# engcang/FAST-LIO-SAM-QN

Measured on AMD Instinct MI355X. Metric: scan-pair registrations/sec on 100k-pt clouds, higher is better.
Workload: dtype f32 search / f64 accumulate

## Files before the change

fast-lio-sam-qn_amd/csrc/qn_knn_hist.cuh:

```cuda
#pragma once
#include "qn_device.cuh"
#include <type_traits>

namespace qn {

#define QN_HB 64
#define QN_HW (QN_HB + 5)
template <int HCAP>
struct WaveLdsH {
  WaveLds s;
  union alignas(16) {
    uint32_t hist[16][QN_HW];
    unsigned long long list[16][HCAP + 1];
    uint4 zero_[(16 * QN_HW + 3) / 4];
  } u;
  uint32_t cnt[16];
  uint32_t kth[16];
  alignas(16) uint32_t tile_sc[64 * 4];
};

typedef float qn_f4v __attribute__((ext_vector_type(4)));
#define QN_MM_FAR 1.0e15f
#define QN_MM_NCH 4
static_assert(QN_MM_NCH == 4, "tile_sc holds 64 x QN_MM_NCH words and is cleared with one 16-byte store per lane; the hit masks are two 32-bit words");
__device__ __forceinline__ uint32_t stage_chunk_mm(const GridView& g, WaveLds* lds, uint32_t* __restrict__ sc_out, const uint32_t cb, const uint32_t total,
                                                   const float Ox, const float Oy, const float Oz, float& c2max, const int j) {
  const int lane = threadIdx.x & 63;
  const uint32_t slot = cb + lane;
  float4 rel = make_float4(QN_MM_FAR, 0.f, 0.f, QN_MM_FAR * QN_MM_FAR); uint32_t sc = 63u << 26;
  if (slot < total) {
    const uint32_t sidx = lds->seg_start[j] + (slot - lds->seg_excl[j]);
    sc = sidx | (lds->seg_cid[j] << 26);
    const float4 p = g.pts[sidx];
    rel.x = p.x - Ox; rel.y = p.y - Oy; rel.z = p.z - Oz; rel.w = (rel.x * rel.x + rel.y * rel.y) + rel.z * rel.z;
    c2max = fmaxf(c2max, rel.w);
  }
  wave_lds_fence();
  lds->tile[lane] = rel; sc_out[lane] = sc;
  wave_lds_fence();
  return min(64u, total - cb);
}

template <int HCAP, bool MM = true>
__device__ __forceinline__ int wave_knn_hist(const GridView& g, float qx, float qy, float qz, bool active, float& r, int k, int max_rounds,
                                             WaveLdsH<HCAP>* L, int32_t* __restrict__ idx_base, float* __restrict__ d2_base, const uint32_t row) {
  const int lane = threadIdx.x & 63, qs = lane & 15, sub = lane >> 4;
  WaveLds* lds = &L->s;
  const int cx = cell_coord(qx, g.ox, g.inv_cell, g.nx);
  const int cy = cell_coord(qy, g.oy, g.inv_cell, g.ny);
  const int cz = cell_coord(qz, g.oz, g.inv_cell, g.nz);
  const float INF = __int_as_float(0x7f800000);
  int status = active ? 1 : 0;
  unsigned long long todo = __ballot(active);
  for (int round = 0; todo != 0 && round < max_rounds; round++) {
    const bool mine = (todo >> lane) & 1ull;
    uint32_t cid; int ncl; uint32_t nseg_all;
    build_clusters<4>(g, lds, todo, cx, cy, cz, qx, qy, qz, r, cid, ncl, nseg_all);
    { uint4* hz = (uint4*)&L->u.hist[0][0];
#pragma unroll
      for (int e = 0; e < (16 * QN_HW + 3) / 4; e += 64) if (e + lane < (16 * QN_HW + 3) / 4) hz[e + lane] = make_uint4(0u, 0u, 0u, 0u); }
    wave_lds_fence();
    const int base = (int)(__float_as_uint(4.f * r * r) >> 20) - (QN_HB - 2);
    const bool one_cluster = ncl == 1;
    const int base1 = mine ? base : -(1 << 28);
    uint32_t ncand;
    float Ox = 0.f, Oy = 0.f, Oz = 0.f, bsel = 0.f, q2 = 0.f, c2max = 0.f;
    if constexpr (MM) {
      const int l0 = __ffsll((long long)todo) - 1;
      Ox = rdlane(qx, l0); Oy = rdlane(qy, l0); Oz = rdlane(qz, l0);
      const float rx = qx - Ox, ry = qy - Oy, rz = qz - Oz;
      q2 = (rx * rx + ry * ry) + rz * rz;
      bsel = sub == 0 ? -2.f * rx : (sub == 1 ? -2.f * ry : (sub == 2 ? -2.f * rz : 1.f));
    }
    const float* tilef = (const float*)&lds->tile[0];
    const qn_f4v cin = {q2, q2, q2, q2};
    auto mm_groups = [&](const float (&av)[4], const uint32_t cnt, auto&& per_group) __attribute__((always_inline)) {
      qn_f4v d = __builtin_amdgcn_mfma_f32_16x16x4f32(av[0], bsel, cin, 0, 0, 0);
#pragma unroll
      for (int gi = 0; gi < 4; gi++) {
        qn_f4v dn = d;
        if (gi < 3) dn = __builtin_amdgcn_mfma_f32_16x16x4f32(av[gi + 1], bsel, cin, 0, 0, 0);
        if ((uint32_t)(16 * gi) < cnt) per_group(gi, d);
        d = dn;
      }
    };
    auto load_av = [&](float (&av)[4]) __attribute__((always_inline)) {
#pragma unroll
      for (int gi = 0; gi < 4; gi++) av[gi] = tilef[(16 * gi + qs) * 4 + sub];
    };
    const bool cached = nseg_all <= 64u && one_cluster;
    float avc[QN_MM_NCH][4];
    if constexpr (MM) {
      auto p1_group = [&](const uint32_t* __restrict__ scb, const int gi, const qn_f4v d) __attribute__((always_inline)) {
        if (one_cluster) {
#pragma unroll
          for (int e = 0; e < 4; e++) {
            const int bin = min(max((__float_as_int(d[e]) >> 20) - base1, 0), QN_HB - 1);
            atomicAdd(&L->u.hist[qs][bin], 1u);
          }
        } else {
          const uint4 cc = *(const uint4*)&scb[16 * gi + 4 * sub];
          const uint32_t ccv[4] = {cc.x >> 26, cc.y >> 26, cc.z >> 26, cc.w >> 26};
#pragma unroll
          for (int e = 0; e < 4; e++) {
            const int bin = max((__float_as_int(d[e]) >> 20) - base, 0);
            const bool ok = mine && ccv[e] == cid && bin < QN_HB - 1;
            atomicAdd(&L->u.hist[qs][ok ? bin : QN_HB + sub], 1u);
          }
        }
      };
      ncand = stream_tables<false>(g, lds, ncl, nseg_all, [&](const uint32_t total) __attribute__((always_inline)) {
        uint32_t cb0 = 0u;
        if (cached) {
          ((uint4*)L->tile_sc)[lane] = make_uint4(0u, 0u, 0u, 0u);
          wave_lds_fence();
          { const uint32_t ex = lds->seg_excl[lane], nx = lane < 63 ? lds->seg_excl[(lane + 1) & 63] : total;
            if (nx > ex && ex < 64u * QN_MM_NCH) L->tile_sc[ex] = (uint32_t)lane + 1u; }
          wave_lds_fence();
          uint32_t carry = 0u;
#pragma unroll
          for (int c = 0; c < QN_MM_NCH; c++) {
            if ((uint32_t)(64 * c) < total) {
              const uint32_t mk = max(wave_incl_max_u32(L->tile_sc[64 * c + lane]), carry);
              carry = rdlane(mk, 63);
              const uint32_t cnt = stage_chunk_mm(g, lds, L->tile_sc + 64 * c, 64u * c, total, Ox, Oy, Oz, c2max, (int)mk - 1);
              load_av(avc[c]);
              mm_groups(avc[c], cnt, [&](const int, const qn_f4v d) __attribute__((always_inline)) {
#pragma unroll
                for (int e = 0; e < 4; e++) atomicAdd(&L->u.hist[qs][min(max((__float_as_int(d[e]) >> 20) - base1, 0), QN_HB - 1)], 1u);
              });
            }
          }
          cb0 = 64u * QN_MM_NCH;
        }
        const uint32_t exs = lds->seg_excl[lane], nxs = lane < 63 ? lds->seg_excl[(lane + 1) & 63] : total;
        for (uint32_t cb = cb0; cb < total; cb += 64) {
          const int jg = chunk_segment(lds->tile_cid, cb, exs, nxs);
          const uint32_t cnt = stage_chunk_mm(g, lds, lds->tile_cid, cb, total, Ox, Oy, Oz, c2max, jg);
          float av[4]; load_av(av);
          mm_groups(av, cnt, [&](const int gi, const qn_f4v d) __attribute__((always_inline)) { p1_group(lds->tile_cid, gi, d); });
        }
      });
    } else {
    auto bin_of = [&](const float4& cp) __attribute__((always_inline)) { return max((int)(__float_as_uint(sqdist(qx, qy, qz, cp.x, cp.y, cp.z)) >> 20) - base, 0); };
    ncand = one_cluster
      ? stream_clusters<4>(g, lds, ncl, nseg_all, [&](const float4& cp, bool, uint32_t) __attribute__((always_inline)) {
          const int bin = min(max((int)(__float_as_uint(sqdist(qx, qy, qz, cp.x, cp.y, cp.z)) >> 20) - base1, 0), QN_HB - 1);
          atomicAdd(&L->u.hist[qs][bin], 1u);
        })
      : stream_clusters<4>(g, lds, ncl, nseg_all, [&](const float4& cp, bool in_tile, uint32_t ccid) __attribute__((always_inline)) {
          const int bin = bin_of(cp);
          const bool ok = mine && in_tile && ccid == cid && bin < QN_HB - 1;
          atomicAdd(&L->u.hist[qs][ok ? bin : QN_HB + sub], 1u);
        });
    }
    wave_lds_fence();
    uint32_t hv[16], mysum = 0;
#pragma unroll
    for (int j = 0; j < 16; j++) { hv[j] = L->u.hist[qs][sub * 16 + j]; if (j == 15 && sub == 3) hv[j] = 0u; mysum += hv[j]; }
    const uint32_t s0 = __shfl(mysum, qs), s1 = __shfl(mysum, qs + 16), s2 = __shfl(mysum, qs + 32), s3 = __shfl(mysum, qs + 48);
    uint32_t run = (sub > 0 ? s0 : 0u) + (sub > 1 ? s1 : 0u) + (sub > 2 ? s2 : 0u);
    const bool enough = s0 + s1 + s2 + s3 >= (uint32_t)k;
    int cross = 1 << 20;
#pragma unroll
    for (int j = 0; j < 16; j++) { run += hv[j]; if (cross == (1 << 20) && run >= (uint32_t)k) cross = sub * 16 + j; }
    cross = min(cross, __shfl_xor(cross, 16)); cross = min(cross, __shfl_xor(cross, 32));
    const uint32_t tau_bits = (uint32_t)(base + cross + 1) << 20;
    wave_lds_fence();
    if (lane < 16) { L->cnt[lane] = 0; L->kth[lane] = 0x7f800000u; }
    { uint4* lz = (uint4*)&L->u.list[0][0];
      constexpr int NZ = (int)(sizeof(L->u.list) / 16);
      static_assert(sizeof(L->u.list) % 16 == 0, "list rows are cleared with 16-byte stores");
#pragma unroll
      for (int e = 0; e < NZ; e += 64) if (e + lane < NZ) lz[e + lane] = make_uint4(0xffffffffu, 0xffffffffu, 0xffffffffu, 0xffffffffu); }
    wave_lds_fence();
    const bool collect = mine && enough;
    if constexpr (MM) {
      const float R2 = wave_max_f(fmaxf(c2max, mine ? q2 : 0.f));
      const float thr = collect ? (__uint_as_float(tau_bits) + 2.f * (R2 * 1.52587890625e-5f)) * 1.000001f : -__int_as_float(0x7f800000);
      float dummy = 0.f;
      const uint32_t cidm = cid;
      if (cached) {
        uint32_t mw[QN_MM_NCH / 2] = {0u, 0u};
#pragma unroll
        for (int c = 0; c < QN_MM_NCH; c++) {
          uint32_t& m = mw[c >> 1];
          if ((uint32_t)(64 * c) < ncand) {
            const uint32_t cnt = min(64u, ncand - 64u * c);
            qn_f4v d = __builtin_amdgcn_mfma_f32_16x16x4f32(avc[c][0], bsel, cin, 0, 0, 0);
#pragma unroll
            for (int gi = 0; gi < 4; gi++) {
              qn_f4v dn = d;
              if (gi < 3) dn = __builtin_amdgcn_mfma_f32_16x16x4f32(avc[c][gi + 1], bsel, cin, 0, 0, 0);
#pragma unroll
              for (int e = 0; e < 4; e++) m = __builtin_amdgcn_alignbit(m, __float_as_uint(d[e] - thr), 31);
              d = dn;
            }
          } else m <<= 16;
        }
        const uint32_t cntl = (uint32_t)(__popc(mw[0]) + __popc(mw[1]));
        const uint32_t h0 = __shfl(cntl, qs), h1 = __shfl(cntl, qs + 16), h2 = __shfl(cntl, qs + 32), h3 = __shfl(cntl, qs + 48);
        uint32_t pos = (sub > 0 ? h0 : 0u) + (sub > 1 ? h1 : 0u) + (sub > 2 ? h2 : 0u);
        if (sub == 0) L->cnt[qs] = h0 + h1 + h2 + h3;
        while (__any((mw[0] | mw[1]) != 0u)) {
          const bool lo = mw[0] != 0u;
          uint32_t w = lo ? mw[0] : mw[1];
          if (w != 0u) {
            const uint32_t I = (uint32_t)__clz((int)w);
            const uint32_t at = (lo ? 0u : 128u) + ((I >> 4) << 6) + (((I >> 2) & 3u) << 4) + 4u * (uint32_t)sub + (I & 3u);
            if (pos < HCAP) L->u.list[qs][pos] = (unsigned long long)(L->tile_sc[at] & 0x03ffffffu);
            pos++;
            w &= ~(0x80000000u >> I);
            if (lo) mw[0] = w; else mw[1] = w;
          }
        }
        wave_lds_fence();
      }
      if (!cached || ncand > 64u * QN_MM_NCH) {
      stream_tables<true>(g, lds, ncl, nseg_all, [&](const uint32_t total) __attribute__((always_inline)) {
        const uint32_t exs = lds->seg_excl[lane], nxs = lane < 63 ? lds->seg_excl[(lane + 1) & 63] : total;
        for (uint32_t cb = cached ? 64u * QN_MM_NCH : 0u; cb < total; cb += 64) {
          const int jg = chunk_segment(lds->tile_cid, cb, exs, nxs);
          const uint32_t cnt = stage_chunk_mm(g, lds, lds->tile_cid, cb, total, Ox, Oy, Oz, dummy, jg);
          float av[4]; load_av(av);
          mm_groups(av, cnt, [&](const int gi, const qn_f4v d) __attribute__((always_inline)) {
            bool hit[4];
#pragma unroll
            for (int e = 0; e < 4; e++) hit[e] = d[e] < thr;
            const uint4 cc = *(const uint4*)&lds->tile_cid[16 * gi + 4 * sub];
            if (!one_cluster) { hit[0] = hit[0] && (cc.x >> 26) == cidm; hit[1] = hit[1] && (cc.y >> 26) == cidm; hit[2] = hit[2] && (cc.z >> 26) == cidm; hit[3] = hit[3] && (cc.w >> 26) == cidm; }
            const uint32_t scv[4] = {cc.x, cc.y, cc.z, cc.w};
            if (hit[0] || hit[1] || hit[2] || hit[3]) {
#pragma unroll
              for (int e = 0; e < 4; e++) if (hit[e]) {
                const uint32_t pos = atomicAdd(&L->cnt[qs], 1u);
                if (pos < HCAP) L->u.list[qs][pos] = (unsigned long long)(scv[e] & 0x03ffffffu);
              }
            }
          });
        }
      }, ncand);
      }
      wave_lds_fence();
      const uint32_t Pn = min(L->cnt[qs], (uint32_t)HCAP);
      const int pmax = wave_max_i(collect ? (int)Pn : 0);
#pragma unroll
      for (int j = 0; j < HCAP / 4; j++) {
        if (4 * j >= pmax) break;
        const uint32_t slot = (uint32_t)(sub + 4 * j);
        if (collect && slot < Pn) {
          const float4 p = g.pts[(uint32_t)L->u.list[qs][slot]];
          L->u.list[qs][slot] = pack_key(sqdist(qx, qy, qz, p.x, p.y, p.z), __float_as_uint(p.w));
        }
      }
    } else {
    auto collect_one = [&](const float4& cp) __attribute__((always_inline)) {
      const float d2 = sqdist(qx, qy, qz, cp.x, cp.y, cp.z);
      if (collect && __float_as_uint(d2) < tau_bits) {
        const uint32_t pos = atomicAdd(&L->cnt[qs], 1u);
        if (pos < HCAP) L->u.list[qs][pos] = pack_key(d2, __float_as_uint(cp.w));
      }
    };
    if (one_cluster) stream_clusters<4, true>(g, lds, ncl, nseg_all, [&](const float4& cp, bool, uint32_t) __attribute__((always_inline)) { collect_one(cp); }, ncand);
    else stream_clusters<4, true>(g, lds, ncl, nseg_all, [&](const float4& cp, bool in_tile, uint32_t ccid) __attribute__((always_inline)) { if (in_tile && ccid == cid) collect_one(cp); }, ncand);
    }
    wave_lds_fence();
    const uint32_t P = L->cnt[qs];
    const bool ok = collect && P <= HCAP;
    const int maxP = wave_max_i(ok ? (int)P : 0);
    unsigned long long own[HCAP / 4]; int rank[HCAP / 4];
#pragma unroll
    for (int j = 0; j < HCAP / 4; j++) { own[j] = L->u.list[qs][sub + 4 * j]; rank[j] = 0; }
    auto rank_pass = [&](auto NJ) __attribute__((always_inline)) {
      for (int f = 0; f < maxP; f += 4) {
        unsigned long long kf[4];
#pragma unroll
        for (int u = 0; u < 4; u++) kf[u] = L->u.list[qs][min(f + u, HCAP)];
#pragma unroll
        for (int u = 0; u < 4; u++) {
#pragma unroll
          for (int j = 0; j < decltype(NJ)::value; j++) rank[j] += kf[u] < own[j] ? 1 : 0;
        }
      }
    };
    if (HCAP > 32 && maxP > 32) rank_pass(std::integral_constant<int, HCAP / 4>());
    else if (maxP > 28) rank_pass(std::integral_constant<int, 8>());
    else if (maxP > 24) rank_pass(std::integral_constant<int, 7>());
    else rank_pass(std::integral_constant<int, 6>());
#pragma unroll
    for (int j = 0; j < HCAP / 4; j++) if (own[j] != QN_INF_KEY && rank[j] == k - 1) L->kth[qs] = (uint32_t)(own[j] >> 32);
    wave_lds_fence();
    const float kth_d2 = __uint_as_float(L->kth[qs]);
    if (g.dbg && lane == 0) { atomicAdd(&g.dbg[0], (uint32_t)ncl); atomicAdd(&g.dbg[1], ncand); }
    bool retry = false;
    if (mine) {
      const int* b = lds->box[cid];
      const int ex0 = b[0], ex1 = b[1], ey0 = b[2], ey1 = b[3], ez0 = b[4], ez1 = b[5];
      float d = INF;
      if (ex0 > 0) d = fminf(d, qx - (g.ox + ex0 * g.cell));
      if (ex1 < g.nx - 1) d = fminf(d, (g.ox + (ex1 + 1) * g.cell) - qx);
      if (ey0 > 0) d = fminf(d, qy - (g.oy + ey0 * g.cell));
      if (ey1 < g.ny - 1) d = fminf(d, (g.oy + (ey1 + 1) * g.cell) - qy);
      if (ez0 > 0) d = fminf(d, qz - (g.oz + ez0 * g.cell));
      if (ez1 < g.nz - 1) d = fminf(d, (g.oz + (ez1 + 1) * g.cell) - qz);
      const bool whole = d == INF || !(r == r);
      if (!enough) {
        if (whole) status = 2;
        else {
          const uint32_t tot = s0 + s1 + s2 + s3;
          if (4u * tot < (uint32_t)k) {
            int kk = k; asm volatile("" : "+s"(kk));
            r = tot > 0 ? 2.f * r * sqrtf((float)kk / (float)tot) * 1.1f : 4.f * r + g.cell;
          } else { r = 2.f * r + g.cell; retry = true; }
        }
      } else if (!ok) status = 2;
      else {
        d -= g.eps;
        if (whole || (d > 0.f && kth_d2 < d * d)) {
          status = 0;
          uint32_t row_l = row; asm volatile("" : "+v"(row_l));
          int32_t* __restrict__ idx_out = idx_base + (size_t)row_l * k; float* __restrict__ d2_out = d2_base ? d2_base + (size_t)row_l * k : nullptr;
#pragma unroll
          for (int j = 0; j < HCAP / 4; j++) if (own[j] != QN_INF_KEY && rank[j] < k) {
            idx_out[rank[j]] = (int32_t)key_idx(own[j]);
            if (d2_out) d2_out[rank[j]] = key_d2(own[j]);
          }
        } else { r = fmaxf(sqrtf(kth_d2) * 1.000001f + g.eps, r + g.eps); retry = true; }
      }
    }
    todo = __ballot(retry && round + 1 < max_rounds);
    if (g.dbg && lane == 0 && todo) atomicAdd(&g.dbg[3], (uint32_t)__popcll(todo));
  }
  return status;
}


#define QN_HCAP1 128
struct WaveLdsH1 {
  WaveLds s;
  uint32_t hist[QN_HB];
  unsigned long long list[QN_HCAP1];
  uint32_t cnt, kth;
  unsigned long long best;
  uint32_t second, pad;
};

__device__ __forceinline__ int wave_knn_single(const GridView& g, float qx, float qy, float qz, float r, int k, WaveLdsH1* L,
                                               int32_t* __restrict__ idx_out, float* __restrict__ d2_out) {
  const int lane = threadIdx.x & 63;
  const float INF = __int_as_float(0x7f800000);
  if (!(qx == qx) || !(qy == qy) || !(qz == qz) || !(r == r)) return 2;
  const CapBox cap = cap_of(g, qx, qy, qz);
  if (cap.S > 0.f) r = fmaxf(r, sqrtf(cap.S) + 0.5f * g.cell);
  const float r_in = r;
  for (int round = 0; round < 64; round++) {
    const float rx = cap_extent(g, cap, r, 0), ry = cap_extent(g, cap, r, 1), rz = cap_extent(g, cap, r, 2);
    int x0 = rfl(cell_coord(qx - rx, g.ox, g.inv_cell, g.nx)), x1 = rfl(cell_coord(qx + rx, g.ox, g.inv_cell, g.nx));
    int y0 = rfl(cell_coord(qy - ry, g.oy, g.inv_cell, g.ny)), y1 = rfl(cell_coord(qy + ry, g.oy, g.inv_cell, g.ny));
    int z0 = rfl(cell_coord(qz - rz, g.oz, g.inv_cell, g.nz)), z1 = rfl(cell_coord(qz + rz, g.oz, g.inv_cell, g.nz));
    const bool tile_mode = ((x1 >> 3) - (x0 >> 3) + 1) * (y1 - y0 + 1) * (z1 - z0 + 1) > 128;
    if (tile_mode) {
      x0 = (x0 >> 3) << 3; x1 = min(((x1 >> 3) << 3) + 7, g.nx - 1);
      y0 = (y0 >> 2) << 2; y1 = min(((y1 >> 2) << 2) + 3, g.ny - 1);
      z0 = (z0 >> 2) << 2; z1 = min(((z1 >> 2) << 2) + 3, g.nz - 1);
    }
    wave_lds_fence();
    L->hist[lane] = 0; if (lane == 0) { L->cnt = 0; L->kth = 0x7f800000u; }
    wave_lds_fence();
    const int base = (int)(__float_as_uint(4.f * r * r) >> 20) - (QN_HB - 2);
    stream_box(g, x0, x1, y0, y1, z0, z1, tile_mode, &L->s, [&](const float4& p, bool valid, uint32_t) __attribute__((always_inline)) {
      const int bin = max((int)(__float_as_uint(sqdist(qx, qy, qz, p.x, p.y, p.z)) >> 20) - base, 0);
      if (valid && bin < QN_HB - 1) atomicAdd(&L->hist[bin], 1u);
    });
    wave_lds_fence();
    const uint32_t hv = lane < QN_HB - 1 ? L->hist[lane] : 0u;
    const uint32_t cum = wave_incl_scan_u32(hv, lane);
    const uint32_t total = rdlane(cum, 63);
    const bool enough = total >= (uint32_t)k;
    const unsigned long long reach = __ballot(cum >= (uint32_t)k);
    const int cross = reach ? __ffsll((long long)reach) - 1 : QN_HB - 2;
    uint32_t tau_bits = (uint32_t)(base + cross + 1) << 20;
    if (enough && rdlane(cum, cross) > (uint32_t)QN_HCAP1 && cross > 0) {
      const uint32_t below = rdlane(cum, cross - 1), need = (uint32_t)k - below;
      const uint32_t hi20 = (uint32_t)(base + cross);
      wave_lds_fence();
      L->hist[lane] = 0;
      wave_lds_fence();
      stream_box(g, x0, x1, y0, y1, z0, z1, tile_mode, &L->s, [&](const float4& p, bool valid, uint32_t) __attribute__((always_inline)) {
        const uint32_t bits = __float_as_uint(sqdist(qx, qy, qz, p.x, p.y, p.z));
        if (valid && (bits >> 20) == hi20) atomicAdd(&L->hist[(bits >> 14) & 63u], 1u);
      });
      wave_lds_fence();
      const uint32_t cum2 = wave_incl_scan_u32(L->hist[lane], lane);
      const unsigned long long reach2 = __ballot(cum2 >= need);
      const int sub = reach2 ? __ffsll((long long)reach2) - 1 : 63;
      tau_bits = (hi20 << 20) + ((uint32_t)(sub + 1) << 14);
    }
    float d = INF;
    if (x0 > 0) d = fminf(d, cap_face_dist(cap, qx - (g.ox + x0 * g.cell), 0));
    if (x1 < g.nx - 1) d = fminf(d, cap_face_dist(cap, (g.ox + (x1 + 1) * g.cell) - qx, 0));
    if (y0 > 0) d = fminf(d, cap_face_dist(cap, qy - (g.oy + y0 * g.cell), 1));
    if (y1 < g.ny - 1) d = fminf(d, cap_face_dist(cap, (g.oy + (y1 + 1) * g.cell) - qy, 1));
    if (z0 > 0) d = fminf(d, cap_face_dist(cap, qz - (g.oz + z0 * g.cell), 2));
    if (z1 < g.nz - 1) d = fminf(d, cap_face_dist(cap, (g.oz + (z1 + 1) * g.cell) - qz, 2));
    const bool whole = d == INF;
    if (!enough) {
      if (whole) return 2;
      if (r_in > 6.f * g.cell) r += (1.f + round) * g.cell;
      else r = total > 0 ? fmaxf(2.f * r * sqrtf((float)k / (float)total) * 1.1f, r + g.cell) : 2.f * r + g.cell;
      continue;
    }
    stream_box(g, x0, x1, y0, y1, z0, z1, tile_mode, &L->s, [&](const float4& p, bool valid, uint32_t) __attribute__((always_inline)) {
      const float d2 = sqdist(qx, qy, qz, p.x, p.y, p.z);
      if (valid && __float_as_uint(d2) < tau_bits) {
        const uint32_t pos = atomicAdd(&L->cnt, 1u);
        if (pos < QN_HCAP1) L->list[pos] = pack_key(d2, __float_as_uint(p.w));
      }
    });
    wave_lds_fence();
    const uint32_t P = L->cnt;
    if (P > QN_HCAP1) return 2;
    const unsigned long long own0 = (uint32_t)lane < P ? L->list[lane] : QN_INF_KEY, own1 = (uint32_t)lane + 64u < P ? L->list[lane + 64] : QN_INF_KEY;
    int rank0 = 0, rank1 = 0;
    for (uint32_t f = 0; f < P; f++) { const unsigned long long kf = L->list[f]; rank0 += kf < own0 ? 1 : 0; rank1 += kf < own1 ? 1 : 0; }
    if (own0 != QN_INF_KEY && rank0 == k - 1) L->kth = (uint32_t)(own0 >> 32);
    if (own1 != QN_INF_KEY && rank1 == k - 1) L->kth = (uint32_t)(own1 >> 32);
    wave_lds_fence();
    const float kth_d2 = __uint_as_float(L->kth);
    const float df = d - g.eps;
    if (whole || (df > 0.f && kth_d2 < df * df)) {
      if (own0 != QN_INF_KEY && rank0 < k) { idx_out[rank0] = (int32_t)key_idx(own0); if (d2_out) d2_out[rank0] = key_d2(own0); }
      if (own1 != QN_INF_KEY && rank1 < k) { idx_out[rank1] = (int32_t)key_idx(own1); if (d2_out) d2_out[rank1] = key_d2(own1); }
      if (lane == 0) { L->second = 0x7f800000u; }
      wave_lds_fence();
      if (own0 != QN_INF_KEY && rank0 == 0) L->best = own0;
      if (own1 != QN_INF_KEY && rank1 == 0) L->best = own1;
      if (own0 != QN_INF_KEY && rank0 == 1) L->second = (uint32_t)(own0 >> 32);
      if (own1 != QN_INF_KEY && rank1 == 1) L->second = (uint32_t)(own1 >> 32);
      wave_lds_fence();
      return 0;
    }
    r = fmaxf(sqrtf(kth_d2) * 1.000001f + g.eps, r + g.eps);
  }
  return 2;
}

}
```

Measured before the change: 4388.

## Rank kNN candidates with packed f32 clamp-FMA counting and 64-bit fallback

Replaces the 64-bit key comparisons in the candidate ranking loop with packed float operations. A clamped v_pk_fma of own distance times a large constant minus the candidate distance yields a 0/1 indicator, which is accumulated in packed f32 accumulators. Empty list slots are now filled with an +inf distance so the float path orders them last. A checksum of the ranks (sum must equal P(P-1)/2) detects ties or inexact cases and falls back to the original 64-bit comparison pass. This cuts VALU work in the O(P^2) rank loop, at the cost of inline asm complexity and an extra wave reduction per round.

```diff
diff --git a/fast-lio-sam-qn_amd/csrc/qn_knn_hist.cuh b/fast-lio-sam-qn_amd/csrc/qn_knn_hist.cuh
--- a/fast-lio-sam-qn_amd/csrc/qn_knn_hist.cuh
+++ b/fast-lio-sam-qn_amd/csrc/qn_knn_hist.cuh
@@ -5,6 +5,7 @@
 namespace qn {
 
 #define QN_HB 64
+#define QN_LIST_FREE 0x7f800000ffffffffull
 #define QN_HW (QN_HB + 5)
 template <int HCAP>
 struct WaveLdsH {
@@ -172,7 +173,7 @@
       constexpr int NZ = (int)(sizeof(L->u.list) / 16);
       static_assert(sizeof(L->u.list) % 16 == 0, "list rows are cleared with 16-byte stores");
 #pragma unroll
-      for (int e = 0; e < NZ; e += 64) if (e + lane < NZ) lz[e + lane] = make_uint4(0xffffffffu, 0xffffffffu, 0xffffffffu, 0xffffffffu); }
+      for (int e = 0; e < NZ; e += 64) if (e + lane < NZ) lz[e + lane] = make_uint4(0xffffffffu, 0x7f800000u, 0xffffffffu, 0x7f800000u); }
     wave_lds_fence();
     const bool collect = mine && enough;
     if constexpr (MM) {
@@ -268,27 +269,71 @@
     const uint32_t P = L->cnt[qs];
     const bool ok = collect && P <= HCAP;
     const int maxP = wave_max_i(ok ? (int)P : 0);
-    unsigned long long own[HCAP / 4]; int rank[HCAP / 4];
-#pragma unroll
-    for (int j = 0; j < HCAP / 4; j++) { own[j] = L->u.list[qs][sub + 4 * j]; rank[j] = 0; }
-    auto rank_pass = [&](auto NJ) __attribute__((always_inline)) {
+    typedef float qn_f2v __attribute__((ext_vector_type(2)));
+    qn_f2v od[HCAP / 8]; uint32_t oi[HCAP / 4]; int rank[HCAP / 4];
+#pragma unroll
+    for (int j = 0; j < HCAP / 4; j++) {
+      const unsigned long long e = L->u.list[qs][sub + 4 * j];
+      od[j >> 1][j & 1] = key_d2(e); oi[j] = key_idx(e); rank[j] = 0;
+    }
+    auto own_key = [&](const int j) __attribute__((always_inline)) { return ((unsigned long long)__float_as_uint(od[j >> 1][j & 1]) << 32) | oi[j]; };
+    auto rank_pass32 = [&](auto NJ) __attribute__((always_inline)) {
+      constexpr int np = (decltype(NJ)::value + 1) / 2;
+      const qn_f2v big = {0x1p100f, 0x1p100f}, nbig = {-0x1p100f, -0x1p100f};
+      qn_f2v acc[np];
+#pragma unroll
+      for (int p = 0; p < np; p++) acc[p] = (qn_f2v){0.f, 0.f};
       for (int f = 0; f < maxP; f += 4) {
         unsigned long long kf[4];
 #pragma unroll
         for (int u = 0; u < 4; u++) kf[u] = L->u.list[qs][min(f + u, HCAP)];
 #pragma unroll
         for (int u = 0; u < 4; u++) {
-#pragma unroll
-          for (int j = 0; j < decltype(NJ)::value; j++) rank[j] += kf[u] < own[j] ? 1 : 0;
-        }
-      }
-    };
-    if (HCAP > 32 && maxP > 32) rank_pass(std::integral_constant<int, HCAP / 4>());
-    else if (maxP > 28) rank_pass(std::integral_constant<int, 8>());
-    else if (maxP > 24) rank_pass(std::integral_constant<int, 7>());
-    else rank_pass(std::integral_constant<int, 6>());
-#pragma unroll
-    for (int j = 0; j < HCAP / 4; j++) if (own[j] != QN_INF_KEY && rank[j] == k - 1) L->kth[qs] = (uint32_t)(own[j] >> 32);
+          qn_f2v nb;
+          asm("v_pk_mul_f32 %0, %1, %2 op_sel:[1,0] op_sel_hi:[1,1]" : "=v"(nb) : "v"(kf[u]), "s"(nbig));
+#pragma unroll
+          for (int p = 0; p < np; p++) {
+            qn_f2v t;
+            asm("v_pk_fma_f32 %0, %1, %2, %3 clamp" : "=v"(t) : "v"(od[p]), "s"(big), "v"(nb));
+            acc[p] += t;
+          }
+        }
+      }
+#pragma unroll
+      for (int j = 0; j < decltype(NJ)::value; j++) rank[j] = (int)acc[j >> 1][j & 1];
+    };
+    auto rank_pass64 = [&](auto NJ) __attribute__((always_inline)) {
+      for (int f = 0; f < maxP; f += 4) {
+        unsigned long long kf[4];
+#pragma unroll
+        for (int u = 0; u < 4; u++) kf[u] = (uint32_t)(f + u) < P ? L->u.list[qs][min(f + u, HCAP)] : QN_INF_KEY;
+#pragma unroll
+        for (int u = 0; u < 4; u++) {
+#pragma unroll
+          for (int j = 0; j < decltype(NJ)::value; j++) rank[j] += kf[u] < own_key(j) ? 1 : 0;
+        }
+      }
+    };
+    auto rank_with = [&](auto&& pass) __attribute__((always_inline)) {
+      if (HCAP > 32 && maxP > 32) pass(std::integral_constant<int, HCAP / 4>());
+      else if (maxP > 28) pass(std::integral_constant<int, 8>());
+      else if (maxP > 24) pass(std::integral_constant<int, 7>());
+      else pass(std::integral_constant<int, 6>());
+    };
+    rank_with(rank_pass32);
+    {
+      int rs = 0;
+#pragma unroll
+      for (int j = 0; j < HCAP / 4; j++) rs += oi[j] != ~0u ? rank[j] : 0;
+      rs += __shfl_xor(rs, 16); rs += __shfl_xor(rs, 32);
+      if (__any(ok && (uint32_t)rs != P * (P - 1u) / 2u)) {
+#pragma unroll
+        for (int j = 0; j < HCAP / 4; j++) rank[j] = 0;
+        rank_with(rank_pass64);
+      }
+    }
+#pragma unroll
+    for (int j = 0; j < HCAP / 4; j++) if (oi[j] != ~0u && rank[j] == k - 1) L->kth[qs] = __float_as_uint(od[j >> 1][j & 1]);
     wave_lds_fence();
     const float kth_d2 = __uint_as_float(L->kth[qs]);
     if (g.dbg && lane == 0) { atomicAdd(&g.dbg[0], (uint32_t)ncl); atomicAdd(&g.dbg[1], ncand); }
@@ -321,9 +366,9 @@
           uint32_t row_l = row; asm volatile("" : "+v"(row_l));
           int32_t* __restrict__ idx_out = idx_base + (size_t)row_l * k; float* __restrict__ d2_out = d2_base ? d2_base + (size_t)row_l * k : nullptr;
 #pragma unroll
-          for (int j = 0; j < HCAP / 4; j++) if (own[j] != QN_INF_KEY && rank[j] < k) {
-            idx_out[rank[j]] = (int32_t)key_idx(own[j]);
-            if (d2_out) d2_out[rank[j]] = key_d2(own[j]);
+          for (int j = 0; j < HCAP / 4; j++) if (oi[j] != ~0u && rank[j] < k) {
+            idx_out[rank[j]] = (int32_t)oi[j];
+            if (d2_out) d2_out[rank[j]] = od[j >> 1][j & 1];
           }
         } else { r = fmaxf(sqrtf(kth_d2) * 1.000001f + g.eps, r + g.eps); retry = true; }
       }
```

Result: no change. 4447 (median of 6 runs) (+1.3%).
